# saegsali/visual-odometry-project

Measured on AMD Instinct MI355X. Metric: VO frames/sec at 1376x1241, 2k keypoints; pose err vs reference, higher is better.
Workload: dtype f64

## Files before the change

### include/vo_hip.h

```cpp
#ifndef VO_HIP_H
#define VO_HIP_H

#include <stddef.h>
#include <stdint.h>

#ifdef __cplusplus
extern "C" {
#endif

typedef struct vo_ctx vo_ctx;

typedef enum vo_status {
  VO_OK = 0,
  VO_EINVAL = -1,
  VO_ENOMEM = -2,
  VO_EHIP = -3,
  VO_ECAPACITY = -4,
  VO_ETRACKING = -5
} vo_status;


int vo_create(int device, void* stream, vo_ctx** out);
void vo_destroy(vo_ctx* ctx);
const char* vo_last_error(const vo_ctx* ctx);
// ... 14 lines not shown
  VO_K_NMS_SELECT = 4,
  VO_K_PATCH_DESC = 5,
  VO_K_PYR_DOWN = 6,
  VO_K_KLT_TRACK = 7,
  VO_K_DLT = 8,
  VO_K_P3P_SOLVE = 9,
  VO_K_P3P_SCORE = 10,
  VO_K_REPROJ = 11,
  VO_K_MATCH = 12,
  VO_K_GATHER = 13,
  VO_K_NMS_ROUND = 14,
  VO_K_NMS_COLLECT = 15,
  VO_K_NMS_RANK = 16,
  VO_K_NMS_EMIT = 17,
  VO_K_SIFT_SCALESPACE = 18,
  VO_K_SIFT_DETECT = 19,
  VO_K_SIFT_DESCRIBE = 20,
  VO_K_REFINE = 21,
  VO_K_STATE_CANDIDATES = 22,
  VO_K_STATE_REGROUP = 23,
  VO_K_RANSAC_REPLAY = 24,
  VO_K_STATE_LANDMARKS = 25,
  VO_K_EXPORT = 26,
  VO_K_COUNT = 32
};
int vo_prof_enable(vo_ctx* ctx, int kernel_id);
int vo_prof_set_sampling(vo_ctx* ctx, int every);
int vo_prof_disable(vo_ctx* ctx);
int vo_prof_read(vo_ctx* ctx, int kernel_id, double* total_ms, int64_t* launches);
int vo_prof_reset(vo_ctx* ctx);
const char* vo_kernel_name(int kernel_id);

int vo_harris_response(vo_ctx* ctx, const uint8_t* img, int H, int W, int patch,
                       double kappa, double* scores);
int vo_harris_keypoints(vo_ctx* ctx, const uint8_t* img, int H, int W, int patch,
                        double kappa, int N, int r, double* kp_xy,
                        double* scores );
int vo_nms_keypoints(vo_ctx* ctx, const double* scores, int H, int W, int N, int r,
                     double* kp_xy);
int vo_harris_keypoints_batch(vo_ctx* ctx, const uint8_t* imgs, int S, int H, int W, int patch, double kappa, int N,
                              int r, double* kp_xy, double* scores );
int vo_harris_response_dev(vo_ctx* ctx, const uint8_t* d_img, int H, int W, int patch,
                           double kappa, double* d_scores);
int vo_nms_keypoints_dev(vo_ctx* ctx, const double* d_scores, int H, int W, int N,
                         int r, double* d_kp_xy);

// ... 172 lines not shown
int vo_pipeline_seed(vo_pipeline* p, const vo_pcg64* rng);
int vo_pipeline_get_rng(vo_pipeline* p, vo_pcg64* rng);
int vo_pipeline_set_state(vo_pipeline* p, int idx, int n, const double* kp, const uint8_t* state,
                          const double* landmarks, const double* tracks, const double* poses,
                          const double* T_wc, const double* T_cw, const double* T_wc_prev,
                          const double* T_cw_prev, int num_features);
int vo_pipeline_set_descriptors(vo_pipeline* p, const float* desc, int n);
int vo_pipeline_set_descriptors_seq(vo_pipeline* p, int seq, const float* desc, int n);
int vo_pipeline_get_descriptors_seq(vo_pipeline* p, int seq, float* desc, int32_t* n_out);
int vo_pipeline_checkpoint(vo_pipeline* p);
int vo_pipeline_rewind(vo_pipeline* p);
int vo_pipeline_feature_cap(vo_pipeline* p);
int vo_pipeline_get_state(vo_pipeline* p, int32_t* n_out, double* kp, uint8_t* state, uint8_t* candidate_mask,
                          double* landmarks, double* tracks, double* poses, double* T_wc, double* T_wc_prev,
                          vo_ransac_state* rs, int32_t* num_features);
int vo_pipeline_get_detection(vo_pipeline* p, double* kp_xy);
int vo_pipeline_step(vo_pipeline* p, int prev_idx, int next_idx, vo_step_result* out);
int vo_pipeline_submit(vo_pipeline* p, int prev_idx, int next_idx);
int vo_pipeline_collect(vo_pipeline* p, vo_step_result* out);
int vo_pipeline_bookkeeping(vo_pipeline* p, int phases, const double* new_kp, int n2, const int32_t* pairs,
                            int M, const double* T_wc, const double* T_cw, const uint8_t* p3p_inliers);
int vo_pipeline_prof_read(vo_pipeline* p, int kernel_id, double* total_ms, int64_t* launches);
int vo_pipeline_prof_reset(vo_pipeline* p);
int vo_pipeline_export_state_post(vo_pipeline* p, const vo_step_result* r, int cap, double* d_record);
int vo_pipeline_export_state_post_seq(vo_pipeline* p, int seq, const vo_step_result* r, int cap, double* d_record);
int vo_pipeline_export_state_join(vo_pipeline* p, void* consumer);
int64_t vo_pipeline_ransac_bound(vo_pipeline* p, double outlier_ratio);
int vo_pipeline_sequences(vo_pipeline* p);
int vo_pipeline_set_frame_seq(vo_pipeline* p, int seq, int idx, const uint8_t* img);
int vo_pipeline_set_frame_pinned(vo_pipeline* p, int seq, int idx, const uint8_t* pinned_img);
int vo_pipeline_frame_uploaded(vo_pipeline* p, int idx, int wait);
int vo_pipeline_prepare(vo_pipeline* p, int idx);
int vo_host_alloc(vo_ctx* ctx, size_t bytes, void** out);
int vo_host_free(vo_ctx* ctx, void* p);
int vo_pipeline_set_state_seq(vo_pipeline* p, int seq, int idx, int n, const double* kp, const uint8_t* state,
                              const double* landmarks, const double* tracks, const double* poses,
                              const double* T_wc, const double* T_cw, const double* T_wc_prev,
                              const double* T_cw_prev, int num_features);
int vo_pipeline_get_state_seq(vo_pipeline* p, int seq, int32_t* n_out, double* kp, uint8_t* state,
                              uint8_t* candidate_mask, double* landmarks, double* tracks, double* poses,
                              double* T_wc, double* T_wc_prev, vo_ransac_state* rs, int32_t* num_features);
int vo_pipeline_get_rng_seq(vo_pipeline* p, int seq, vo_pcg64* rng);
int vo_pipeline_collect_all(vo_pipeline* p, vo_step_result* outs);
int vo_pipeline_set_camera_seq(vo_pipeline* p, int seq, const double K[9], const double Kinv[9]);
int vo_pipeline_set_active_seq(vo_pipeline* p, int seq, int active);
int vo_pipeline_restart_seq(vo_pipeline* p, int seq, int idx, int n, const double* kp, const uint8_t* state,
// ... 44 lines not shown
```

### visual-odometry-project_amd/csrc/klt.hip

```cpp
#include "vo_internal.h"

#pragma clang fp contract(off)

namespace {

constexpr int MAX_LEVELS = 8;
constexpr int MAX_WIN = 31;
constexpr int W_BITS = 14;

constexpr int PYR_PAD = 32;

struct pyr_t {
  const uint8_t* prev[MAX_LEVELS];
  const uint8_t* next[MAX_LEVELS];
  int H[MAX_LEVELS], W[MAX_LEVELS], pitch[MAX_LEVELS];
  int n_levels;
};

__host__ __device__ inline int pyr_pitch(int W) { return (W + 2 * PYR_PAD + 3) & ~3; }
inline size_t pyr_level_bytes(int H, int W) {
  return ((size_t)(H + 2 * PYR_PAD) * pyr_pitch(W) + 255) & ~size_t(255);
}

__device__ __forceinline__ int reflect101(int c, int n) {
// ... 385 lines not shown
    }
#pragma unroll
    for (int k = 0; k < 8; ++k) {
      const int i = b0 + k * 64 + lane;
      if (i < total) s[i] = v[k];
    }
  }
}

constexpr int KLT_MARGIN = 4;
constexpr int KLT_WAVES = 4;

__device__ __forceinline__ void wave_sync() {
  __builtin_amdgcn_fence(__ATOMIC_SEQ_CST, "wavefront");
  __builtin_amdgcn_wave_barrier();
}

template <int WIN_T>
__global__ __launch_bounds__(64 * KLT_WAVES) void klt_track_kernel(pyr_t P, const float* __restrict__ prev_xy, int N, const int* __restrict__ d_n, vo_klt_source src, vo_klt_batch B, int win_arg,
                                                       int max_iter, double eps2, float min_eig_thr,
                                                       float* __restrict__ next_xy, uint8_t* __restrict__ status,
                                                       float* __restrict__ err, int lds_per_wave) {
  extern __shared__ __align__(16) unsigned char smem_all[];
  const int i = blockIdx.x * KLT_WAVES + (threadIdx.x >> 6);
  size_t pyr_off = 0;
  if (blockIdx.y != 0) {
    const size_t q = blockIdx.y;
    pyr_off = q * B.pyr;
    prev_xy += q * B.xy;
    next_xy += q * B.xy;
    status += q * B.out;
    err += q * B.out;
    if (src.n) {
      src.n = reinterpret_cast<const int32_t*>(reinterpret_cast<const char*>(src.n) + q * B.ctl);
      src.num_features = reinterpret_cast<const int32_t*>(reinterpret_cast<const char*>(src.num_features) + q * B.ctl);
      src.det_kp += q * B.det;
      if (src.ts) src.ts = reinterpret_cast<unsigned long long*>(reinterpret_cast<char*>(src.ts) + q * B.ctl);
      if (src.det_go) src.det_go += q;
    }
  }
  if (d_n) N = min(N, *d_n);
  int n_own = N;
  if (src.ts && blockIdx.x == 0 && threadIdx.x == 0) *src.ts = wall_clock64();
  if (src.n) {
    n_own = *src.n;
    const bool redetect = (double)n_own < (double)*src.num_features * src.frac && (!src.det_go || *src.det_go != 0);
    N = min(N, n_own + (redetect ? src.n_det : 0));
  }
  if (i >= N) return;
  unsigned char* smem = smem_all + (size_t)(threadIdx.x >> 6) * lds_per_wave;
  const int lane = threadIdx.x & 63;
  const int win = WIN_T > 0 ? WIN_T : win_arg;
  const int ww = win * win;
  const int n1 = win + 1, n3 = win + 3;
  const int RS = n1 + 2 * KLT_MARGIN;
  uint8_t* s_reg = smem;
  int* s_der = reinterpret_cast<int*>(smem + ((max(n3 * n3, RS * RS) + 15) & ~15));
  short4* s_tpl = reinterpret_cast<short4*>(s_der + n1 * n1 + ((n1 * n1) & 1));

  const float half = (float)(win - 1) * 0.5f;
  const float FLT_SCALE = 1.f / (float)(1 << 20);
  const float p0x = i < n_own ? prev_xy[2 * i] : (float)src.det_kp[2 * (i - n_own)];
  const float p0y = i < n_own ? prev_xy[2 * i + 1] : (float)src.det_kp[2 * (i - n_own) + 1];
  bool ok = true;
  float e_out = 0.f;
  float nx = 0.f, ny = 0.f;

  for (int level = P.n_levels - 1; level >= 0; --level) {
    const uint8_t* I = P.prev[level] + pyr_off;
    const uint8_t* J = P.next[level] + pyr_off;
    const int H = P.H[level], W = P.W[level], pitch = P.pitch[level];
// ... 244 lines not shown
      unsigned* d = reinterpret_cast<unsigned*>(s + row * PITCH);
#pragma unroll
      for (int k = 0; k < b.WORDS; ++k) d[k] = b.v[pass][k];
    }
  }
}
template <int NC, int NR, int LPK, int PITCH>
__device__ __forceinline__ void stage16(const uint8_t* __restrict__ img, int pitch, int x0, int y0, uint8_t* s, int r) {
  staged_block<NC, NR, LPK> b;
  stage_load<NC, NR, LPK>(img, pitch, x0, y0, r, b);
  stage_store<NC, NR, LPK, PITCH>(b, s, r);
}

template <int WIN, int LPK>
__global__ __launch_bounds__(64) void klt_track16_kernel(pyr_t P, const float* __restrict__ prev_xy, int N, const int* __restrict__ d_n, vo_klt_source src, vo_klt_batch B, int max_iter,
                                                         double eps2, float min_eig_thr, float* __restrict__ next_xy,
                                                         uint8_t* __restrict__ status, float* __restrict__ err) {
  typedef klt_rows<WIN> G;
  constexpr int win = WIN, ww = WIN * WIN, RS = G::RS, n1 = G::n1, n3 = G::n3, K16_PITCH = G::PITCH;
  constexpr int KPW = 64 / LPK;
  static_assert(n1 <= LPK, "one lane per derivative row");
  __shared__ __align__(16) uint8_t smem[KPW * G::SLICE + 16];
  const int lane = threadIdx.x;
  const int i = blockIdx.x * KPW + lane / LPK;
  size_t pyr_off = 0;
  if (blockIdx.y != 0) {
    const size_t q = blockIdx.y;
    pyr_off = q * B.pyr;
    prev_xy += q * B.xy;
    next_xy += q * B.xy;
    status += q * B.out;
    err += q * B.out;
    if (src.n) {
      src.n = reinterpret_cast<const int32_t*>(reinterpret_cast<const char*>(src.n) + q * B.ctl);
      src.num_features = reinterpret_cast<const int32_t*>(reinterpret_cast<const char*>(src.num_features) + q * B.ctl);
      src.det_kp += q * B.det;
      if (src.ts) src.ts = reinterpret_cast<unsigned long long*>(reinterpret_cast<char*>(src.ts) + q * B.ctl);
      if (src.det_go) src.det_go += q;
    }
  }
  if (d_n) N = min(N, *d_n);
  int n_own = N;
  if (src.ts && blockIdx.x == 0 && threadIdx.x == 0) *src.ts = wall_clock64();
  if (src.n) {
    n_own = *src.n;
    const bool redetect = (double)n_own < (double)*src.num_features * src.frac && (!src.det_go || *src.det_go != 0);
    N = min(N, n_own + (redetect ? src.n_det : 0));
  }
  if (i >= N) return;
  const int r = lane & (LPK - 1);
  uint8_t* s_reg = smem + (lane / LPK) * G::SLICE;
  const int live = r < win ? 1 : 0;
  const int rr = r < win ? r : win - 1;
  const int rd = r < n1 ? r : n1 - 1;

  const float half = (float)(win - 1) * 0.5f;
  const float FLT_SCALE = 1.f / (float)(1 << 20);
  float p0x, p0y;
  if (i >= n_own) {
    p0x = (float)src.det_kp[2 * (i - n_own)];
    p0y = (float)src.det_kp[2 * (i - n_own) + 1];
  } else {
    p0x = prev_xy[2 * i];
    p0y = prev_xy[2 * i + 1];
  }
  bool ok = true;
  float e_out = 0.f;
  float nx = 0.f, ny = 0.f;

  staged_block<n3, n3, LPK> tplI;
  auto request_template = [&](int level) {
// ... 342 lines not shown
  VO_HIP_TRY(ctx, hipSetDevice(ctx->device));
  pyr_t P;
  memset(&P, 0, sizeof(P));
  P.n_levels = n_levels;
  {
    size_t off = 0;
    int h = H, w = W;
    for (int l = 0; l < n_levels; ++l) {
      P.H[l] = h;
      P.W[l] = w;
      P.pitch[l] = pyr_pitch(w);
      const size_t origin = off + (size_t)PYR_PAD * P.pitch[l] + PYR_PAD;
      P.prev[l] = d_prev_pyr + origin;
      P.next[l] = d_next_pyr + origin;
      off += pyr_level_bytes(h, w);
      h = (h + 1) / 2;
      w = (w + 1) / 2;
    }
  }
  if (max_iter < 0) max_iter = 0;
  if (max_iter > 100) max_iter = 100;
  if (eps < 0) eps = 0;
  if (eps > 10) eps = 10;
  {
    vo_prof_scope ps(ctx, VO_K_KLT_TRACK);
    const int lds_wave = (int)((klt_lds_bytes(win) + 15) & ~size_t(15));
    const size_t lds = (size_t)lds_wave * KLT_WAVES;
    hipStream_t st = ctx->stream;
    const float me = (float)min_eig;
    const dim3 kgrid(vo_cdiv(N, KLT_WAVES), S), kblock(64 * KLT_WAVES);
    switch (win) {
      case 15:
        vo_launch_stop(ctx, klt_track16_kernel<15, 16>, dim3(vo_cdiv(N, 4), S), dim3(64), 0, st, P, d_prev_xy, N, d_n, src, B,
                       max_iter, eps * eps, me, d_next_xy, d_status, d_err);
        break;
      case 17:
        vo_launch_stop(ctx, klt_track16_kernel<17, 32>, dim3(vo_cdiv(N, 2), S), dim3(64), 0, st, P, d_prev_xy, N, d_n, src, B,
                       max_iter, eps * eps, me, d_next_xy, d_status, d_err);
        break;
      case 21:
        vo_launch_stop(ctx, klt_track16_kernel<21, 32>, dim3(vo_cdiv(N, 2), S), dim3(64), 0, st, P, d_prev_xy, N, d_n, src, B,
                       max_iter, eps * eps, me, d_next_xy, d_status, d_err);
        break;
      default:
        vo_launch_stop(ctx, klt_track_kernel<0>, kgrid, kblock, lds, st, P, d_prev_xy, N, d_n, src, B, win, max_iter, eps * eps,
                       me, d_next_xy, d_status, d_err, lds_wave);
    }
  }
  return vo_check_launch(ctx, "klt_track_kernel");
}

extern "C" {

int vo_klt_track(vo_ctx* ctx, const uint8_t* prev, const uint8_t* next, int H, int W, const float* prev_xy, int N,
                 int win, int max_level, int max_iter, double eps, double min_eig, float* next_xy, uint8_t* status,
                 float* err) {
  if (!ctx) return VO_EINVAL;
  VO_REQUIRE(ctx, N >= 0, "klt_track: bad N");
  if (N == 0) return VO_OK;
  VO_REQUIRE(ctx, prev && next && prev_xy && next_xy && status && err, "klt_track: null pointer");
  VO_REQUIRE(ctx, H > 0 && W > 0 && max_level >= 0, "klt_track: bad arguments");
  VO_REQUIRE(ctx, win >= 3 && win <= MAX_WIN, "klt_track: window must be in 3..%d", MAX_WIN);
  const int nl = vo_klt_num_levels(H, W, win, max_level);
  const size_t px = (size_t)H * W, pb = vo_pyramid_bytes(H, W, nl);
// ... 46 lines not shown
```

### visual-odometry-project_amd/csrc/pipeline.h

```cpp
#pragma once

#include <linux/futex.h>
#include <sys/prctl.h>
#include <sys/syscall.h>
#include <time.h>
#include <unistd.h>

#include <atomic>
#include <chrono>
#include <cmath>
#include <cstdlib>
#include <string>
#include <mutex>
#include <thread>
#include <vector>

#include "vo_state.h"
#include "state_device.h"

struct vo_pipeline_boot;

struct vo_pipeline {
  vo_ctx* ctx = nullptr;
  vo_ctx* det = nullptr;
// ... 65 lines not shown
  uint8_t* d_frame_desc = nullptr;
  int32_t* d_frame_n = nullptr;
  uint8_t* d_fdesc = nullptr;
  int32_t* d_srcrow = nullptr;
  uint8_t* d_ckpt_fdesc = nullptr;
  char* d_ckpt_feat = nullptr;
  vo_seq_ctl* d_ckpt_ctl = nullptr;
  size_t feat_block = 0;
  int ckpt_frame = -1;
  int32_t* d_pairs = nullptr;
  long n_recovered = 0, n_continued = 0;
  bool pose_fault_hook = true;
  std::thread worker;
  std::atomic<unsigned> job_posted{0}, job_done{0};
  std::atomic<int> worker_asleep{0};
  std::atomic<bool> quit{false};
  int threads_budget = 2;
  double spin_s = 150e-6;
  vo_stream_cfg side_cfg;
  int desc_chains_pending = 0;
  flight_t jobs[4];
  int worker_rc = 0;
  char worker_err[256] = {0};
  double dbg_part[4] = {0, 0, 0, 0};
  double dbg_submit = 0, dbg_wait = 0;
  long dbg_steps = 0;
  std::vector<void*> dev_mem, host_mem;
  std::vector<hipEvent_t> events;

  uint8_t* img(int q, int idx) const { return d_img + ((size_t)q * cfg.n_frames + idx) * px; }
  size_t img_stride() const { return (size_t)cfg.n_frames * px; }
  uint8_t* pyr(int q, int s) const { return d_pyr + ((size_t)q * 3 + s) * pyr_bytes; }
  size_t pyr_stride() const { return 3 * pyr_bytes; }
  double* kp(int q, int s) const { return d_kp + ((size_t)q * 3 + s) * cfg.n_keypoints * 2; }
  size_t det_stride() const { return (size_t)3 * cfg.n_keypoints * 2; }
  vo_step_result* res_h(int rslot, int q) const { return h_res + (size_t)rslot * S + q; }
  uint8_t* frame_desc(int s, int q) const { return d_frame_desc + ((size_t)s * S + q) * frame_rows * desc_row; }
  uint8_t* fdesc(int fb, int q) const { return d_fdesc + ((size_t)fb * S + q) * cap * desc_row; }
  int32_t* frame_n(int s, int q) const { return d_frame_n + (size_t)s * S + q; }
  int32_t* npairs(int q) const { return d_frame_n + (size_t)3 * S + q; }
  volatile unsigned* seq_h(int rslot, int q) const { return h_seq + (size_t)rslot * S + q; }
};


template <typename T>
static inline int dev_alloc(vo_pipeline* p, T** out, size_t count) {
// ... 82 lines not shown
```

### visual-odometry-project_amd/csrc/pipeline.hip

```cpp
#include "pipeline.h"

#pragma clang fp contract(off)

namespace {

hipError_t mset(hipStream_t st, void* dst, int v, size_t bytes) {
  hipError_t e = hipMemsetAsync(dst, v, bytes, st);
  return e != hipSuccess ? e : hipStreamSynchronize(st);
}

uint32_t next_pow2(uint64_t v) {
  uint32_t r = 1;
  while (r < v) r <<= 1;
  return r;
}

vo_feat carve(char*& q, int cap, int S) {
  vo_feat f;
  auto take = [&](size_t bytes) {
    void* r = q;
    q += (bytes * S + 255) & ~size_t(255);
    return r;
  };
  f.kp = (float*)take((size_t)cap * 8);
// ... 161 lines not shown
  p->ctx = ctx;
  p->cfg = *cfg;
  p->cap = cap;
  p->words = vo_cdiv(cap, 64);
  p->S = cfg->sequences > 0 ? cfg->sequences : 1;
  p->cfg.sequences = p->S;
  const int S = p->S;
  if (p->cfg.bearing_threshold == 0.0) p->cfg.bearing_threshold = 0.0075;
  if (p->cfg.redetect_fraction == 0.0) p->cfg.redetect_fraction = 0.8;
  if (p->cfg.detect_margin == 0.0) p->cfg.detect_margin = 0.01;
  if (p->cfg.detect_losses <= 0.0) p->cfg.detect_losses = 2.5;
  p->detect_losses = p->cfg.detect_losses;
  p->detect_limit = p->cfg.detect_margin < 0.0 ? -1.0 : p->cfg.redetect_fraction + p->cfg.detect_margin;
  if (p->cfg.debug_never_detect) p->detect_limit = 0.0;
  {
    bool given = false;
    for (double v : cfg->Kinv) given |= v != 0.0;
    p->cams.assign((size_t)p->S, make_cam(cfg->K, given ? cfg->Kinv : nullptr));
  }
  p->idle.assign((size_t)p->S, 0);
  memset(&p->seed_rng, 0, sizeof(p->seed_rng));
  int rc = VO_OK;
  void* side = getenv("VO_ONE_STREAM") ? (void*)ctx->stream : nullptr;
  {
    const char* sc = getenv("VO_SIDE_CUS");
    p->side_cfg = vo_stream_cfg_parse(sc, getenv("VO_STREAM_PRIORITY"));
    if (!sc && p->S <= 2 && p->detect_limit >= 0.0 && !side && cfg->tracker_mode == 0) {
      hipDeviceProp_t prop;
      if (hipGetDeviceProperties(&prop, ctx->device) == hipSuccess && prop.multiProcessorCount >= 128) {
        p->side_cfg.cu_lo = 32;
        p->side_cfg.cu_hi = prop.multiProcessorCount - 1;
      }
    }
    if (!side && side_pool_evicts()) side_evict_except(ctx->device, p->side_cfg);
    for (vo_ctx** c : {&p->trk, &p->det})
      if ((side ? vo_create_stream(ctx->device, side, p->side_cfg, c) : side_take(ctx->device, p->side_cfg, c)) != VO_OK)
        rc = vo_set_error(ctx, VO_EHIP, "pipeline: cannot create the side streams");
  }
  dbg_stage("create: side streams made");
  const int N = cfg->n_keypoints, Hyp = cfg->hyp;
  const size_t px = (size_t)cfg->H * cfg->W, Sz = (size_t)S;
  p->px = px;
  p->n_levels = vo_klt_num_levels(cfg->H, cfg->W, cfg->klt_win, cfg->klt_max_level);
  p->pyr_bytes = vo_pyramid_bytes(cfg->H, cfg->W, p->n_levels);
#define PA(expr) do { if (rc == VO_OK) rc = (expr); } while (0)
  PA(dev_alloc(p, &p->d_img, Sz * cfg->n_frames * px));
// ... 227 lines not shown
  VO_TRY(worker_idle(p));
  double sum = 0;
  int64_t n = 0;
  for (vo_ctx* q : {p->ctx, p->det, p->trk}) {
    double ms = 0;
    int64_t k = 0;
    const int rc = vo_prof_read(q, kernel_id, &ms, &k);
    if (rc != VO_OK) return q == p->ctx ? rc : vo_set_error(p->ctx, rc, "%s", vo_last_error(q));
    sum += ms;
    n += k;
  }
  if (total_ms) *total_ms = sum;
  if (launches) *launches = n;
  return VO_OK;
}

int vo_pipeline_prof_reset(vo_pipeline* p) {
  if (!p) return VO_EINVAL;
  VO_TRY(worker_idle(p));
  for (vo_ctx* q : {p->ctx, p->det, p->trk}) VO_TRY(vo_prof_reset(q));
  return VO_OK;
}

}
```

### visual-odometry-project_amd/csrc/pipeline_step.hip

```cpp
#include "pipeline.h"

#pragma clang fp contract(off)

namespace {

__global__ __launch_bounds__(64) void detect_decide_kernel(const vo_seq_ctl* __restrict__ ctl, int S, double limit, int n_det,
                                                           int force, int* __restrict__ go, double losses) {
  const int q = blockIdx.x * 64 + threadIdx.x;
  if (q >= S) return;
  if (ctl[q].fault & VO_FAULT_IDLE) {
    go[q] = 0;
    return;
  }
  const int n2 = ctl[q].n2;
  const int lost = max(ctl[q].n_in - (ctl[q].redetected ? n_det : 0) - n2, 0);
  go[q] = (force || limit < 0.0 || (limit > 0.0 && (double)n2 - losses * (double)lost < (double)ctl[q].num_features * limit)) ? 1 : 0;
}

__global__ void ctl_resume_kernel(vo_seq_ctl* __restrict__ ctl) {
  ctl->fault = 0;
  ctl->n_p3p = ctl->n_tri;
}

__global__ __launch_bounds__(256) void sift_kp_f64_kernel(const float* __restrict__ rows, const int* __restrict__ n, int cap,
// ... 132 lines not shown
  j.rp.t = p->d_t + q * c.hyp * 3;
  j.rp.masks = (const unsigned long long*)p->d_masks + q * c.hyp * p->words;
  j.rp.words = p->words;
  j.rp.hyp = c.hyp;
  j.rp.table = p->d_table;
  j.rp.table_len = p->table_len;
  j.rp.max_it = c.ransac_max_iterations;
  j.rp.best_mask = (unsigned long long*)p->d_best_mask + q * p->words;
  j.do_replay = do_replay;
  j.B = vo_feat_seq(B, q);
  j.cam = p->d_cams + q;
  j.bearing_thr = c.bearing_threshold;
  j.max_iter = c.refine_iters;
  j.tail = 0;
  j.res = nullptr;
  j.seq_word = nullptr;
  j.seq = 0u;
  static const int stamps = getenv("VO_POSE_STAMPS") ? 1 : 0;
  j.stamps = stamps;
  j.debug_fault_every = 0;
  return j;
}

static int enqueue_tracker(vo_pipeline* p, const vo_pipeline::flight_t& f, bool with_pyramid, int q0, int Sn) {
  vo_ctx* ctx = p->ctx;
  const vo_pipeline_config& c = p->cfg;
  const vo_feat A = vo_feat_seq(p->F[f.fcur], (size_t)q0);
  hipStream_t ts = p->trk->stream;
  if (with_pyramid) VO_TRY(enqueue_pyramid(p, f.next_idx, f.b));
  if (f.k > 0 && hipEventQuery(p->evRegroup[(f.k - 1) & 1]) != hipSuccess)
    VO_HIP_TRY(ctx, hipStreamWaitEvent(ts, p->evRegroup[(f.k - 1) & 1], 0));
  if (hipEventQuery(p->evDet[f.a]) != hipSuccess) VO_HIP_TRY(ctx, hipStreamWaitEvent(ts, p->evDet[f.a], 0));
  vo_seq_ctl* ctl = p->d_ctl + q0;
  vo_klt_source src;
  src.n = &ctl->n2;
  src.num_features = &ctl->num_features;
  src.frac = c.redetect_fraction;
  src.det_kp = p->kp(q0, f.a);
  src.n_det = c.n_keypoints;
  src.ts = &ctl->ts[0];
  src.det_go = p->d_det_go + (size_t)f.a * p->S + q0;
  vo_klt_batch kb;
  kb.S = Sn;
  kb.pyr = p->pyr_stride();
  kb.xy = (size_t)p->cap * 2;
  kb.out = (size_t)p->cap;
  kb.ctl = sizeof(vo_seq_ctl);
  kb.det = p->det_stride();
  p->trk->next_stop = p->evKlt[f.k & 1];
  {
    const size_t q = (size_t)q0;
    const int rc = vo_klt_track_ndev(p->trk, p->img(q0, f.prev_idx), p->pyr(q0, f.a), p->img(q0, f.next_idx), p->pyr(q0, f.b),
                                     c.H, c.W, p->n_levels, A.kp, p->cap, nullptr, c.klt_win, c.klt_max_iter, c.klt_eps,
                                     c.klt_min_eig, p->d_next + q * p->cap * 2, p->d_status + q * p->cap,
                                     p->d_err + q * p->cap, &src, &kb);
    if (rc != VO_OK) return vo_set_error(ctx, rc, "tracker: %s", vo_last_error(p->trk));
  }
  if (p->trk->next_stop) {
    p->trk->next_stop = nullptr;
    VO_HIP_TRY(ctx, hipEventRecord(p->evKlt[f.k & 1], ts));
  }
  return VO_OK;
}

static int enqueue_pose_half(vo_pipeline* p, const vo_pipeline::flight_t& f, int q0, int Sn, unsigned seq);

static int enqueue_chain(vo_pipeline* p, const vo_pipeline::flight_t& f, bool first_half_only, int debug_fault_every,
                         int q0, int Sn, unsigned seq) {
  vo_ctx* ctx = p->ctx;
  const vo_pipeline_config& c = p->cfg;
  const size_t q = (size_t)q0;
  const vo_feat A = vo_feat_seq(p->F[f.fcur], q), B = vo_feat_seq(p->F[1 - f.fcur], q);
  vo_seq_ctl* ctl = p->d_ctl + q0;
  VO_HIP_TRY(ctx, hipStreamWaitEvent(ctx->stream, p->evKlt[f.k & 1], 0));
  vo_append ap;
  ap.det_kp = p->kp(q0, f.a);
  ap.det_stride = p->det_stride();
  ap.n_det = c.n_keypoints;
  ap.frac = c.redetect_fraction;
  ap.pose_mode = c.redetect_start_pose;
// ... 271 lines not shown
      }
    }
    for (int q = 0; q < p->S; ++q) p->slot_seq[(size_t)f.rslot * p->S + q] = f.seq;
    p->flight[p->n_flight++] = f;
    ++p->desc_chains_pending;
    VO_TRY(flush_desc_chains(p));
  } else {
    double tq = now_s();
    const bool detect_early = p->detect_limit < 0.0;
    if (p->threads_budget >= 2) {
      const unsigned my = p->job_posted.load(std::memory_order_relaxed);
      wait_until(50e-6, [&] { return (int)(p->job_done.load(std::memory_order_acquire) - my) >= 0; });
      VO_TRY(worker_check(p));
      sync_prof(p);
      if (detect_early) post_job(p, f);
    } else {
      sync_prof(p);
    }
    double tn = now_s();
    p->dbg_part[0] += tn - tq;
    tq = tn;
    const bool have_pyr = p->prepared_idx == next_idx && p->prepared_slot == f.b;
    p->prepared_idx = p->prepared_slot = -1;
    VO_TRY(enqueue_tracker(p, f, !have_pyr, 0, p->S));
    tn = now_s();
    p->dbg_part[1] += tn - tq;
    tq = tn;
    for (int q = 0; q < p->S; ++q) VO_TRY(ensure_raws(p, q));
    tn = now_s();
    p->dbg_part[2] += tn - tq;
    tq = tn;
    VO_TRY(enqueue_chain(p, f, false, c.debug_fault_every, 0, p->S, f.seq));
    for (int q = 0; q < p->S; ++q) p->slot_seq[(size_t)f.rslot * p->S + q] = f.seq;
    if (p->threads_budget < 2) VO_TRY(enqueue_detection(p, f.next_idx, f.b, false));
    else if (!detect_early) post_job(p, f);
    p->dbg_part[3] += now_s() - tq;
    p->flight[p->n_flight++] = f;
  }
  ++p->steps_submitted;
  p->slot = f.b;
  p->cur = 1 - f.fcur;
  p->prev_frame = next_idx;
  p->dbg_submit += now_s() - t_in;
  ++p->dbg_steps;
  return VO_OK;
}

// ... 288 lines not shown
```

### visual-odometry-project_amd/csrc/vo_ctx.hip

```cpp
#include "vo_internal.h"

int vo_set_error(vo_ctx* ctx, int code, const char* fmt, ...) {
  if (ctx) {
    va_list ap;
    va_start(ap, fmt);
    vsnprintf(ctx->err, sizeof(ctx->err), fmt, ap);
    va_end(ap);
  }
  return code;
}

int vo_ensure(vo_ctx* ctx, vo_buf& b, size_t bytes) {
  if (bytes <= b.cap) return VO_OK;
  VO_HIP_TRY(ctx, hipSetDevice(ctx->device));
  VO_HIP_TRY(ctx, hipStreamSynchronize(ctx->stream));
  if (b.p) VO_HIP_TRY(ctx, hipFree(b.p));
  b.p = nullptr;
  b.cap = 0;
  size_t want = (bytes + 255) & ~size_t(255);
  hipError_t e = hipMalloc(&b.p, want);
  if (e != hipSuccess) {
    b.p = nullptr;
    return vo_set_error(ctx, VO_ENOMEM, "hipMalloc(%zu) failed: %s", want, hipGetErrorString(e));
  }
// ... 132 lines not shown
}

int vo_dev_upload(vo_ctx* ctx, void* dst, const void* src, size_t bytes) {
  if (!ctx || (!dst && bytes) || (!src && bytes)) return VO_EINVAL;
  if (!bytes) return VO_OK;
  VO_HIP_TRY(ctx, hipMemcpyAsync(dst, src, bytes, hipMemcpyHostToDevice, ctx->stream));
  VO_HIP_TRY(ctx, hipStreamSynchronize(ctx->stream));
  return VO_OK;
}

int vo_dev_download(vo_ctx* ctx, void* dst, const void* src, size_t bytes) {
  if (!ctx || (!dst && bytes) || (!src && bytes)) return VO_EINVAL;
  if (!bytes) return VO_OK;
  VO_HIP_TRY(ctx, hipMemcpyAsync(dst, src, bytes, hipMemcpyDeviceToHost, ctx->stream));
  VO_HIP_TRY(ctx, hipStreamSynchronize(ctx->stream));
  return VO_OK;
}


static const char* const k_names[VO_K_COUNT] = {
    "harris_response", "nms_candidates", "nms_threshold", "nms_compact", "nms_select",
    "patch_descriptors", "pyr_down", "klt_track", "dlt_triangulate", "p3p_solve",
    "p3p_score", "reproj_inliers", "match_knn2", "track_gather", "nms_round", "nms_collect", "nms_rank", "nms_emit", "sift_scale_space", "sift_detect", "sift_describe", "refine_pose",
    "state_candidates", "state_regroup", "ransac_replay", "state_landmarks", "export_state"};

const char* vo_kernel_name(int k) {
  if (k < 0 || k >= VO_K_COUNT || !k_names[k]) return "";
  return k_names[k];
}

int vo_prof_enable(vo_ctx* ctx, int kernel_id) {
  if (!ctx || kernel_id >= VO_K_COUNT) return VO_EINVAL;
  ctx->prof_on = true;
  ctx->prof_kernel = kernel_id;
  return VO_OK;
}

int vo_prof_set_sampling(vo_ctx* ctx, int every) {
  if (!ctx || every < 1) return VO_EINVAL;
  ctx->prof_every = every;
  return VO_OK;
}

int vo_prof_disable(vo_ctx* ctx) {
  if (!ctx) return VO_EINVAL;
  ctx->prof_on = false;
  return VO_OK;
// ... 62 lines not shown
```

### visual-odometry-project_amd/csrc/vo_internal.h

```cpp
#pragma once
#include <hip/hip_runtime.h>
#include <hip/hip_ext.h>

#include <cstdarg>
#include <cstdint>
#include <cstdio>
#include <cstdlib>
#include <cstring>
#include <vector>

#include "vo_hip.h"

struct vo_buf {
  void* p = nullptr;
  size_t cap = 0;
};

struct vo_prof_slot {
  double total_ms = 0.0;
  int64_t launches = 0;
};

struct vo_prof_pair {
  int k;
// ... 168 lines not shown
  int32_t status;
  int32_t n, best_count, consumed, finished_by_host;
  int64_t iterations;
};
int vo_fundamental_ransac_dev(vo_ctx* ctx, const double* d_p1, const double* d_p2, int n_cap, const int32_t* d_n,
                              const int32_t* n_host, const vo_f8_params& prm, vo_pcg64* rngs, uint8_t* d_inl, double* d_F,
                              const vo_f8_lanes* lanes, vo_f8_result* res);
int vo_relative_pose_lanes_dev(vo_ctx* ctx, const double* d_x1, const double* d_x2, const vo_f8_lanes& lanes, const uint8_t* d_inl,
                               const double* d_F, const double* d_cam, size_t cam_stride, const int32_t* d_seq, double* d_M,
                               double* d_X, size_t X_stride, uint8_t* d_mask_out);
int vo_triangulate_dlt_ndev(vo_ctx* ctx, const double* d_x1, const double* d_x2, const int32_t* d_n, int n_cap,
                            const double* d_C1, const double* d_C2, double* d_X);
int vo_refine_pose_ndev(vo_ctx* ctx, const double* d_X, const double* d_x, int N, const int32_t* d_n, const double* K,
                        const uint8_t* d_mask8, const uint64_t* d_mask_bits, const double* d_Rt0, int max_iter,
                        double* d_out14, unsigned tag);
struct vo_klt_source {
  const int32_t* n = nullptr;
  const int32_t* num_features = nullptr;
  double frac = 0.0;
  const double* det_kp = nullptr;
  int n_det = 0;
  unsigned long long* ts = nullptr;
  const int* det_go = nullptr;
};
struct vo_klt_batch {
  int S = 1;
  size_t pyr = 0;
  size_t xy = 0;
  size_t out = 0;
  size_t ctl = 0;
  size_t det = 0;
};
int vo_klt_track_ndev(vo_ctx* ctx, const uint8_t* d_prev, const uint8_t* d_prev_pyr, const uint8_t* d_next,
                      const uint8_t* d_next_pyr, int H, int W, int n_levels, const float* d_prev_xy, int N,
                      const int32_t* d_n, int win, int max_iter, double eps, double min_eig, float* d_next_xy,
                      uint8_t* d_status, float* d_err, const vo_klt_source* src = nullptr,
                      const vo_klt_batch* batch = nullptr);
int vo_pyramid_build_batch_dev(vo_ctx* ctx, const uint8_t* d_img, size_t img_stride, int S, int H, int W, int n_levels,
                               uint8_t* d_pyr, size_t pyr_stride);
int vo_harris_response_batch_dev(vo_ctx* ctx, const uint8_t* d_img, size_t img_stride, int S, int H, int W, int patch,
                                 double kappa, double* d_scores, const int* d_go = nullptr);
int vo_nms_keypoints_batch_dev(vo_ctx* ctx, const double* d_scores, int S, int H, int W, int N, int r, double* d_kp_xy,
                               size_t kp_stride, const int* d_go = nullptr);
```

### visual-odometry-project_amd/vo/_native.py

```python
import ctypes as C
import atexit
import os
import threading
import weakref

import numpy as np

_LIB_PATH = os.path.join(os.path.dirname(os.path.abspath(__file__)), "lib", "libvo_hip.so")

VO_OK, VO_EINVAL, VO_ENOMEM, VO_EHIP, VO_ECAPACITY, VO_ETRACKING = 0, -1, -2, -3, -4, -5
_CODES = {VO_EINVAL: "VO_EINVAL", VO_ENOMEM: "VO_ENOMEM", VO_EHIP: "VO_EHIP", VO_ECAPACITY: "VO_ECAPACITY",
          VO_ETRACKING: "VO_ETRACKING"}

K_HARRIS_RESPONSE, K_NMS_CANDIDATES, K_NMS_THRESHOLD, K_NMS_COMPACT, K_NMS_SELECT = 0, 1, 2, 3, 4
K_PATCH_DESC, K_PYR_DOWN, K_KLT_TRACK, K_DLT, K_P3P_SOLVE, K_P3P_SCORE, K_REPROJ, K_MATCH = 5, 6, 7, 8, 9, 10, 11, 12
K_COUNT = 32


class VoError(RuntimeError):
    def __init__(self, code, msg):
        super().__init__("%s (%d): %s" % (_CODES.get(code, "VO_E?"), code, msg))
        self.code = code


_lib = None
_lib_lock = threading.Lock()


class Pcg64(C.Structure):
    _fields_ = [("state_hi", C.c_uint64), ("state_lo", C.c_uint64), ("inc_hi", C.c_uint64), ("inc_lo", C.c_uint64),
                ("has_uint32", C.c_uint32), ("uinteger", C.c_uint32)]

    @classmethod
    def from_generator(cls, gen):
        st = gen.bit_generator.state
        assert st["bit_generator"] == "PCG64"
        s, inc = st["state"]["state"], st["state"]["inc"]
        m = (1 << 64) - 1
# ... 143 lines not shown
    "vo_pipeline_set_descriptors": (_i, [_vp, _vp, _i]),
    "vo_pipeline_set_descriptors_seq": (_i, [_vp, _i, _vp, _i]),
    "vo_pipeline_get_descriptors_seq": (_i, [_vp, _i, _vp, _vp]),
    "vo_pipeline_checkpoint": (_i, [_vp]),
    "vo_pipeline_rewind": (_i, [_vp]),
    "vo_pipeline_destroy": (None, [_vp]),
    "vo_pipeline_release_cached": (None, []),
    "vo_pipeline_release_cached_at_exit": (_i, []),
    "vo_pipeline_set_frame": (_i, [_vp, _i, _vp]),
    "vo_pipeline_seed": (_i, [_vp, _vp]),
    "vo_pipeline_get_rng": (_i, [_vp, _vp]),
    "vo_pipeline_set_state": (_i, [_vp, _i, _i, _vp, _vp, _vp, _vp, _vp, _vp, _vp, _vp, _vp, _i]),
    "vo_pipeline_feature_cap": (_i, [_vp]),
    "vo_pipeline_get_state": (_i, [_vp, _vp, _vp, _vp, _vp, _vp, _vp, _vp, _vp, _vp, _vp, _vp]),
    "vo_pipeline_get_detection": (_i, [_vp, _vp]),
    "vo_pipeline_step": (_i, [_vp, _i, _i, _vp]),
    "vo_pipeline_submit": (_i, [_vp, _i, _i]),
    "vo_pipeline_collect": (_i, [_vp, _vp]),
    "vo_pipeline_bookkeeping": (_i, [_vp, _i, _vp, _i, _vp, _i, _vp, _vp, _vp]),
    "vo_pipeline_export_state_post": (_i, [_vp, _vp, _i, _vp]),
    "vo_pipeline_export_state_join": (_i, [_vp, _vp]),
    "vo_pipeline_prof_read": (_i, [_vp, _i, C.POINTER(_d), C.POINTER(C.c_int64)]),
    "vo_pipeline_prof_reset": (_i, [_vp]),
    "vo_pipeline_ransac_bound": (C.c_int64, [_vp, _d]),
    "vo_pipeline_sequences": (_i, [_vp]),
    "vo_pipeline_set_frame_seq": (_i, [_vp, _i, _i, _vp]),
    "vo_pipeline_set_frame_pinned": (_i, [_vp, _i, _i, _vp]),
    "vo_pipeline_frame_uploaded": (_i, [_vp, _i, _i]),
    "vo_pipeline_prepare": (_i, [_vp, _i]),
    "vo_host_alloc": (_i, [_vp, C.c_size_t, C.POINTER(C.c_void_p)]),
    "vo_host_free": (_i, [_vp, _vp]),
    "vo_pipeline_set_state_seq": (_i, [_vp, _i, _i, _i, _vp, _vp, _vp, _vp, _vp, _vp, _vp, _vp, _vp, _i]),
    "vo_pipeline_get_state_seq": (_i, [_vp, _i, _vp, _vp, _vp, _vp, _vp, _vp, _vp, _vp, _vp, _vp, _vp]),
    "vo_pipeline_get_rng_seq": (_i, [_vp, _i, _vp]),
    "vo_pipeline_collect_all": (_i, [_vp, _vp]),
    "vo_pipeline_export_state_post_seq": (_i, [_vp, _i, _vp, _i, _vp]),
    "vo_pipeline_set_camera_seq": (_i, [_vp, _i, _vp, _vp]),
    "vo_pipeline_set_active_seq": (_i, [_vp, _i, _i]),
    "vo_pipeline_restart_seq": (_i, [_vp, _i, _i, _i, _vp, _vp, _vp, _vp, _vp, _vp, _vp, _vp, _vp, _i, _vp]),
    "vo_pipeline_bootstrap_seq": (_i, [_vp, _i, _i, _i, _vp, _vp, _vp]),
    "vo_pipeline_bootstrap": (_i, [_vp, _i, _i, _vp, _vp]),
    "vo_pipeline_bootstrap_lanes": (_i, [_vp, _i, _vp, _i, _i, _vp, _vp, _vp, _vp]),
    "vo_bootstrap_default_rng": (None, [_vp]),
}


# ... 583 lines not shown
```

### visual-odometry-project_amd/vo/_pipeline.py

```python
import ctypes as C

import numpy as np


def _ptr(a):
    return a.ctypes.data_as(C.c_void_p) if a is not None else None


def _c(a, dtype):
    return np.ascontiguousarray(a, dtype=dtype)


def _as_4x4(pose):
    pose = np.asarray(pose, np.float64)
    if pose.shape == (3, 4):
        pose = np.vstack([pose, [0.0, 0.0, 0.0, 1.0]])
    return np.ascontiguousarray(pose)


class Pipeline:
    def __init__(self, ctx, H, W, n_frames, K, n_keypoints=2000, harris_patch=9, harris_kappa=0.09, nms_radius=5,
                 klt_win=15, klt_max_level=2, klt_max_iter=10, klt_eps=0.03, klt_min_eig=1e-4,
                 klt_err_threshold=100.0, hyp=1000, p3p_threshold=1.0, outlier_ratio=0.9, confidence=0.99,
                 max_iterations=1000, seed=2023, refine_iters=0, feature_cap=0, bearing_threshold=0.0075,
# ... 231 lines not shown
    def bookkeeping(self, phases, new_keypoints=None, pairs=None, pose_world_cam=None, p3p_inliers=None):
        if phases & 1:
            kp = _c(np.asarray(new_keypoints).reshape(-1, 2), np.float64)
            pr = _c(np.asarray(pairs).reshape(-1, 2), np.int32)
            T_wc = _as_4x4(pose_world_cam)
            T_cw = _c(np.linalg.inv(T_wc), np.float64)
            inl = None if p3p_inliers is None else _c(np.asarray(p3p_inliers).reshape(-1), np.uint8)
            self.ctx._chk(self.ctx._lib.vo_pipeline_bookkeeping(self._h, int(phases), _ptr(kp), kp.shape[0], _ptr(pr),
                                                                pr.shape[0], _ptr(T_wc), _ptr(T_cw), _ptr(inl)))
        else:
            self.ctx._chk(self.ctx._lib.vo_pipeline_bookkeeping(self._h, int(phases), None, 0, None, 0, None, None, None))

    def ransac_bound(self, outlier_ratio):
        return int(self.ctx._lib.vo_pipeline_ransac_bound(self._h, float(outlier_ratio)))

    def prof_read(self, kernel_id):
        ms, n = C.c_double(), C.c_int64()
        self.ctx._chk(self.ctx._lib.vo_pipeline_prof_read(self._h, int(kernel_id), C.byref(ms), C.byref(n)))
        return ms.value, n.value

    def prof_reset(self):
        self.ctx._chk(self.ctx._lib.vo_pipeline_prof_reset(self._h))

    def export_state_post(self, result, cap, d_record, seq=0):
        self.ctx._chk(self.ctx._lib.vo_pipeline_export_state_post_seq(self._h, int(seq), C.byref(result), int(cap),
                                                                      C.c_void_p(d_record)))

    def export_state_join(self, consumer_stream=None):
        self.ctx._chk(self.ctx._lib.vo_pipeline_export_state_join(self._h, C.c_void_p(consumer_stream or 0)))
```

Baseline: 10870.

## Split KLT tracking so existing tracks start before redetection finishes

When the detection event is still pending, the tracker now launches in two parts. First it tracks only the existing keypoints without waiting on detection. After the stream waits on the detection event, a second append launch tracks the newly detected keypoints. This is meant to overlap existing-track KLT with the detection work instead of serialising them, at the cost of an extra kernel launch and a possible second partially-filled grid.

```diff
diff --git a/include/vo_hip.h b/include/vo_hip.h
--- a/include/vo_hip.h
+++ b/include/vo_hip.h
@@ -60,6 +60,7 @@
   VO_K_RANSAC_REPLAY = 24,
   VO_K_STATE_LANDMARKS = 25,
   VO_K_EXPORT = 26,
+  VO_K_KLT_APPEND = 27,
   VO_K_COUNT = 32
 };
 int vo_prof_enable(vo_ctx* ctx, int kernel_id);
@@ -278,6 +279,7 @@
                             int M, const double* T_wc, const double* T_cw, const uint8_t* p3p_inliers);
 int vo_pipeline_prof_read(vo_pipeline* p, int kernel_id, double* total_ms, int64_t* launches);
 int vo_pipeline_prof_reset(vo_pipeline* p);
+int64_t vo_pipeline_tracker_split_steps(vo_pipeline* p);
 int vo_pipeline_export_state_post(vo_pipeline* p, const vo_step_result* r, int cap, double* d_record);
 int vo_pipeline_export_state_post_seq(vo_pipeline* p, int seq, const vo_step_result* r, int cap, double* d_record);
 int vo_pipeline_export_state_join(vo_pipeline* p, void* consumer);
diff --git a/visual-odometry-project_amd/csrc/klt.hip b/visual-odometry-project_amd/csrc/klt.hip
--- a/visual-odometry-project_amd/csrc/klt.hip
+++ b/visual-odometry-project_amd/csrc/klt.hip
@@ -431,7 +431,7 @@
                                                        float* __restrict__ next_xy, uint8_t* __restrict__ status,
                                                        float* __restrict__ err, int lds_per_wave) {
   extern __shared__ __align__(16) unsigned char smem_all[];
-  const int i = blockIdx.x * KLT_WAVES + (threadIdx.x >> 6);
+  int i0 = blockIdx.x * KLT_WAVES + (threadIdx.x >> 6);
   size_t pyr_off = 0;
   if (blockIdx.y != 0) {
     const size_t q = blockIdx.y;
@@ -450,12 +450,21 @@
   }
   if (d_n) N = min(N, *d_n);
   int n_own = N;
-  if (src.ts && blockIdx.x == 0 && threadIdx.x == 0) *src.ts = wall_clock64();
+  if (src.ts && src.part != 2 && blockIdx.x == 0 && threadIdx.x == 0) *src.ts = wall_clock64();
   if (src.n) {
     n_own = *src.n;
-    const bool redetect = (double)n_own < (double)*src.num_features * src.frac && (!src.det_go || *src.det_go != 0);
-    N = min(N, n_own + (redetect ? src.n_det : 0));
-  }
+    if (src.part == 1) {
+      N = min(N, n_own);
+    } else {
+      const bool redetect = (double)n_own < (double)*src.num_features * src.frac && (!src.det_go || *src.det_go != 0);
+      if (src.part == 2) {
+        if (!redetect) return;
+        i0 += n_own;
+      }
+      N = min(N, n_own + (redetect ? src.n_det : 0));
+    }
+  }
+  const int i = i0;
   if (i >= N) return;
   unsigned char* smem = smem_all + (size_t)(threadIdx.x >> 6) * lds_per_wave;
   const int lane = threadIdx.x & 63;
@@ -746,7 +755,7 @@
   static_assert(n1 <= LPK, "one lane per derivative row");
   __shared__ __align__(16) uint8_t smem[KPW * G::SLICE + 16];
   const int lane = threadIdx.x;
-  const int i = blockIdx.x * KPW + lane / LPK;
+  int i0 = blockIdx.x * KPW + lane / LPK;
   size_t pyr_off = 0;
   if (blockIdx.y != 0) {
     const size_t q = blockIdx.y;
@@ -765,12 +774,21 @@
   }
   if (d_n) N = min(N, *d_n);
   int n_own = N;
-  if (src.ts && blockIdx.x == 0 && threadIdx.x == 0) *src.ts = wall_clock64();
+  if (src.ts && src.part != 2 && blockIdx.x == 0 && threadIdx.x == 0) *src.ts = wall_clock64();
   if (src.n) {
     n_own = *src.n;
-    const bool redetect = (double)n_own < (double)*src.num_features * src.frac && (!src.det_go || *src.det_go != 0);
-    N = min(N, n_own + (redetect ? src.n_det : 0));
-  }
+    if (src.part == 1) {
+      N = min(N, n_own);
+    } else {
+      const bool redetect = (double)n_own < (double)*src.num_features * src.frac && (!src.det_go || *src.det_go != 0);
+      if (src.part == 2) {
+        if (!redetect) return;
+        i0 += n_own;
+      }
+      N = min(N, n_own + (redetect ? src.n_det : 0));
+    }
+  }
+  const int i = i0;
   if (i >= N) return;
   const int r = lane & (LPK - 1);
   uint8_t* s_reg = smem + (lane / LPK) * G::SLICE;
@@ -1159,24 +1177,27 @@
   if (max_iter > 100) max_iter = 100;
   if (eps < 0) eps = 0;
   if (eps > 10) eps = 10;
+  VO_REQUIRE(ctx, src.part >= 0 && src.part <= 2 && (src.part == 0 || src.n), "klt_track: bad part");
+  const int G = src.part == 2 ? (src.n_det < N ? src.n_det : N) : N;
+  if (G <= 0) return VO_OK;
   {
-    vo_prof_scope ps(ctx, VO_K_KLT_TRACK);
+    vo_prof_scope ps(ctx, src.part == 2 ? VO_K_KLT_APPEND : VO_K_KLT_TRACK);
     const int lds_wave = (int)((klt_lds_bytes(win) + 15) & ~size_t(15));
     const size_t lds = (size_t)lds_wave * KLT_WAVES;
     hipStream_t st = ctx->stream;
     const float me = (float)min_eig;
-    const dim3 kgrid(vo_cdiv(N, KLT_WAVES), S), kblock(64 * KLT_WAVES);
+    const dim3 kgrid(vo_cdiv(G, KLT_WAVES), S), kblock(64 * KLT_WAVES);
     switch (win) {
       case 15:
-        vo_launch_stop(ctx, klt_track16_kernel<15, 16>, dim3(vo_cdiv(N, 4), S), dim3(64), 0, st, P, d_prev_xy, N, d_n, src, B,
+        vo_launch_stop(ctx, klt_track16_kernel<15, 16>, dim3(vo_cdiv(G, 4), S), dim3(64), 0, st, P, d_prev_xy, N, d_n, src, B,
                        max_iter, eps * eps, me, d_next_xy, d_status, d_err);
         break;
       case 17:
-        vo_launch_stop(ctx, klt_track16_kernel<17, 32>, dim3(vo_cdiv(N, 2), S), dim3(64), 0, st, P, d_prev_xy, N, d_n, src, B,
+        vo_launch_stop(ctx, klt_track16_kernel<17, 32>, dim3(vo_cdiv(G, 2), S), dim3(64), 0, st, P, d_prev_xy, N, d_n, src, B,
                        max_iter, eps * eps, me, d_next_xy, d_status, d_err);
         break;
       case 21:
-        vo_launch_stop(ctx, klt_track16_kernel<21, 32>, dim3(vo_cdiv(N, 2), S), dim3(64), 0, st, P, d_prev_xy, N, d_n, src, B,
+        vo_launch_stop(ctx, klt_track16_kernel<21, 32>, dim3(vo_cdiv(G, 2), S), dim3(64), 0, st, P, d_prev_xy, N, d_n, src, B,
                        max_iter, eps * eps, me, d_next_xy, d_status, d_err);
         break;
       default:
diff --git a/visual-odometry-project_amd/csrc/pipeline.h b/visual-odometry-project_amd/csrc/pipeline.h
--- a/visual-odometry-project_amd/csrc/pipeline.h
+++ b/visual-odometry-project_amd/csrc/pipeline.h
@@ -111,6 +111,8 @@
   flight_t jobs[4];
   int worker_rc = 0;
   char worker_err[256] = {0};
+  int tracker_split = 2;
+  long n_split_steps = 0;
   double dbg_part[4] = {0, 0, 0, 0};
   double dbg_submit = 0, dbg_wait = 0;
   long dbg_steps = 0;
diff --git a/visual-odometry-project_amd/csrc/pipeline.hip b/visual-odometry-project_amd/csrc/pipeline.hip
--- a/visual-odometry-project_amd/csrc/pipeline.hip
+++ b/visual-odometry-project_amd/csrc/pipeline.hip
@@ -207,6 +207,8 @@
   memset(&p->seed_rng, 0, sizeof(p->seed_rng));
   int rc = VO_OK;
   void* side = getenv("VO_ONE_STREAM") ? (void*)ctx->stream : nullptr;
+  if (const char* ts = getenv("VO_TRACKER_SPLIT"))
+    p->tracker_split = strcmp(ts, "never") == 0 ? 0 : strcmp(ts, "always") == 0 ? 1 : 2;
   {
     const char* sc = getenv("VO_SIDE_CUS");
     p->side_cfg = vo_stream_cfg_parse(sc, getenv("VO_STREAM_PRIORITY"));
@@ -480,4 +482,6 @@
   return VO_OK;
 }
 
-}
+int64_t vo_pipeline_tracker_split_steps(vo_pipeline* p) { return p ? (int64_t)p->n_split_steps : -1; }
+
+}
diff --git a/visual-odometry-project_amd/csrc/pipeline_step.hip b/visual-odometry-project_amd/csrc/pipeline_step.hip
--- a/visual-odometry-project_amd/csrc/pipeline_step.hip
+++ b/visual-odometry-project_amd/csrc/pipeline_step.hip
@@ -178,7 +178,8 @@
   return j;
 }
 
-static int enqueue_tracker(vo_pipeline* p, const vo_pipeline::flight_t& f, bool with_pyramid, int q0, int Sn) {
+static int enqueue_tracker(vo_pipeline* p, const vo_pipeline::flight_t& f, bool with_pyramid, int q0, int Sn,
+                           bool* split_out = nullptr) {
   vo_ctx* ctx = p->ctx;
   const vo_pipeline_config& c = p->cfg;
   const vo_feat A = vo_feat_seq(p->F[f.fcur], (size_t)q0);
@@ -186,7 +187,10 @@
   if (with_pyramid) VO_TRY(enqueue_pyramid(p, f.next_idx, f.b));
   if (f.k > 0 && hipEventQuery(p->evRegroup[(f.k - 1) & 1]) != hipSuccess)
     VO_HIP_TRY(ctx, hipStreamWaitEvent(ts, p->evRegroup[(f.k - 1) & 1], 0));
-  if (hipEventQuery(p->evDet[f.a]) != hipSuccess) VO_HIP_TRY(ctx, hipStreamWaitEvent(ts, p->evDet[f.a], 0));
+  const bool det_pending = p->tracker_split != 1 && hipEventQuery(p->evDet[f.a]) != hipSuccess;
+  const bool split = p->tracker_split == 1 || (p->tracker_split == 2 && det_pending);
+  if (split_out) *split_out = split;
+  if (det_pending && !split) VO_HIP_TRY(ctx, hipStreamWaitEvent(ts, p->evDet[f.a], 0));
   vo_seq_ctl* ctl = p->d_ctl + q0;
   vo_klt_source src;
   src.n = &ctl->n2;
@@ -203,15 +207,21 @@
   kb.out = (size_t)p->cap;
   kb.ctl = sizeof(vo_seq_ctl);
   kb.det = p->det_stride();
-  p->trk->next_stop = p->evKlt[f.k & 1];
-  {
-    const size_t q = (size_t)q0;
+  const size_t q = (size_t)q0;
+  auto launch = [&](int part) {
+    src.part = part;
     const int rc = vo_klt_track_ndev(p->trk, p->img(q0, f.prev_idx), p->pyr(q0, f.a), p->img(q0, f.next_idx), p->pyr(q0, f.b),
                                      c.H, c.W, p->n_levels, A.kp, p->cap, nullptr, c.klt_win, c.klt_max_iter, c.klt_eps,
                                      c.klt_min_eig, p->d_next + q * p->cap * 2, p->d_status + q * p->cap,
                                      p->d_err + q * p->cap, &src, &kb);
-    if (rc != VO_OK) return vo_set_error(ctx, rc, "tracker: %s", vo_last_error(p->trk));
-  }
+    return rc != VO_OK ? vo_set_error(ctx, rc, "tracker: %s", vo_last_error(p->trk)) : VO_OK;
+  };
+  if (split) {
+    VO_TRY(launch(1));
+    VO_HIP_TRY(ctx, hipStreamWaitEvent(ts, p->evDet[f.a], 0));
+  }
+  p->trk->next_stop = p->evKlt[f.k & 1];
+  VO_TRY(launch(split ? 2 : 0));
   if (p->trk->next_stop) {
     p->trk->next_stop = nullptr;
     VO_HIP_TRY(ctx, hipEventRecord(p->evKlt[f.k & 1], ts));
@@ -529,7 +539,9 @@
     tq = tn;
     const bool have_pyr = p->prepared_idx == next_idx && p->prepared_slot == f.b;
     p->prepared_idx = p->prepared_slot = -1;
-    VO_TRY(enqueue_tracker(p, f, !have_pyr, 0, p->S));
+    bool split = false;
+    VO_TRY(enqueue_tracker(p, f, !have_pyr, 0, p->S, &split));
+    if (split) ++p->n_split_steps;
     tn = now_s();
     p->dbg_part[1] += tn - tq;
     tq = tn;
diff --git a/visual-odometry-project_amd/csrc/vo_ctx.hip b/visual-odometry-project_amd/csrc/vo_ctx.hip
--- a/visual-odometry-project_amd/csrc/vo_ctx.hip
+++ b/visual-odometry-project_amd/csrc/vo_ctx.hip
@@ -178,7 +178,7 @@
     "harris_response", "nms_candidates", "nms_threshold", "nms_compact", "nms_select",
     "patch_descriptors", "pyr_down", "klt_track", "dlt_triangulate", "p3p_solve",
     "p3p_score", "reproj_inliers", "match_knn2", "track_gather", "nms_round", "nms_collect", "nms_rank", "nms_emit", "sift_scale_space", "sift_detect", "sift_describe", "refine_pose",
-    "state_candidates", "state_regroup", "ransac_replay", "state_landmarks", "export_state"};
+    "state_candidates", "state_regroup", "ransac_replay", "state_landmarks", "export_state", "klt_append"};
 
 const char* vo_kernel_name(int k) {
   if (k < 0 || k >= VO_K_COUNT || !k_names[k]) return "";
diff --git a/visual-odometry-project_amd/csrc/vo_internal.h b/visual-odometry-project_amd/csrc/vo_internal.h
--- a/visual-odometry-project_amd/csrc/vo_internal.h
+++ b/visual-odometry-project_amd/csrc/vo_internal.h
@@ -214,6 +214,7 @@
   int n_det = 0;
   unsigned long long* ts = nullptr;
   const int* det_go = nullptr;
+  int part = 0;
 };
 struct vo_klt_batch {
   int S = 1;
diff --git a/visual-odometry-project_amd/vo/_native.py b/visual-odometry-project_amd/vo/_native.py
--- a/visual-odometry-project_amd/vo/_native.py
+++ b/visual-odometry-project_amd/vo/_native.py
@@ -14,6 +14,7 @@
 
 K_HARRIS_RESPONSE, K_NMS_CANDIDATES, K_NMS_THRESHOLD, K_NMS_COMPACT, K_NMS_SELECT = 0, 1, 2, 3, 4
 K_PATCH_DESC, K_PYR_DOWN, K_KLT_TRACK, K_DLT, K_P3P_SOLVE, K_P3P_SCORE, K_REPROJ, K_MATCH = 5, 6, 7, 8, 9, 10, 11, 12
+K_KLT_APPEND = 27
 K_COUNT = 32
 
 
@@ -203,6 +204,7 @@
     "vo_pipeline_export_state_join": (_i, [_vp, _vp]),
     "vo_pipeline_prof_read": (_i, [_vp, _i, C.POINTER(_d), C.POINTER(C.c_int64)]),
     "vo_pipeline_prof_reset": (_i, [_vp]),
+    "vo_pipeline_tracker_split_steps": (C.c_int64, [_vp]),
     "vo_pipeline_ransac_bound": (C.c_int64, [_vp, _d]),
     "vo_pipeline_sequences": (_i, [_vp]),
     "vo_pipeline_set_frame_seq": (_i, [_vp, _i, _i, _vp]),
diff --git a/visual-odometry-project_amd/vo/_pipeline.py b/visual-odometry-project_amd/vo/_pipeline.py
--- a/visual-odometry-project_amd/vo/_pipeline.py
+++ b/visual-odometry-project_amd/vo/_pipeline.py
@@ -277,6 +277,9 @@
     def prof_reset(self):
         self.ctx._chk(self.ctx._lib.vo_pipeline_prof_reset(self._h))
 
+    def tracker_split_steps(self):
+        return int(self.ctx._lib.vo_pipeline_tracker_split_steps(self._h))
+
     def export_state_post(self, result, cap, d_record, seq=0):
         self.ctx._chk(self.ctx._lib.vo_pipeline_export_state_post_seq(self._h, int(seq), C.byref(result), int(cap),
                                                                       C.c_void_p(d_record)))
```

Result: slower. 10530 (-3.1%).
